# liron88/HM-16.2

Hardware: AMD Instinct MI355X
Metric: CTUs/sec (enc) at 4K main10; bit-exact CU partition vs HM (higher is better)
Workload: dtype int32+f64

## Files before the change

### hm-16.2_amd/csrc/hm355.hip

```cpp
#include <hip/hip_runtime.h>
#include <stdio.h>
#include <stdlib.h>
#include <string.h>
#include <memory>
#include <string>
#include <vector>
#include "hm355_core.h"
#include "hm355_dbk.h"
#include "hm355_sao.h"
#include "hm355_bits_kernel.h"
#include "hm355_ingest.h"
#include "hm355_picstat.h"
#include "hm355_host_common.h"
#include "../../include/hm355.h"

#define HM_SPIN_TIMEOUT_TICKS (40ull * 100000000ull)
typedef __attribute__((address_space(1))) unsigned int gu32;

__device__ __attribute__((noinline)) int hm355_wait_flag(const unsigned int *flag, unsigned int *abortWord, unsigned int epoch)
{
  int bad = 0;
  if (hm_lane() == 0) {
    const gu32 *f = (const gu32 *)flag; gu32 *ab = (gu32 *)abortWord;
    unsigned long long t0 = wall_clock64();
    unsigned int seen = __hip_atomic_load(ab + 1, __ATOMIC_RELAXED, __HIP_MEMORY_SCOPE_AGENT);
    while (__hip_atomic_load(f, __ATOMIC_RELAXED, __HIP_MEMORY_SCOPE_AGENT) != epoch) {
      __builtin_amdgcn_s_sleep(32);
      int stop = __hip_atomic_load(ab, __ATOMIC_RELAXED, __HIP_MEMORY_SCOPE_AGENT) != 0u;
      if (!stop && wall_clock64() - t0 > HM_SPIN_TIMEOUT_TICKS) {
        const unsigned int now = __hip_atomic_load(ab + 1, __ATOMIC_RELAXED, __HIP_MEMORY_SCOPE_AGENT);
        if (now != seen) { seen = now; t0 = wall_clock64(); } else stop = 1;
      }
      if (stop) {
        __hip_atomic_store(ab, 1u, __ATOMIC_RELAXED, __HIP_MEMORY_SCOPE_AGENT);
        bad = 1; break;
      }
    }
  }
  return __shfl(bad, 0, 64);
}

extern "C" __global__ void __launch_bounds__(64 * HM_CTU_WAVES, 3) hm355_ctu_kernel(const Params *P, const WorkItem *items, int total, unsigned int *sched, unsigned int epoch)
{
  __shared__ WorkItem curItems[HM_CTU_WAVES];
  const int wave = __builtin_amdgcn_readfirstlane((int)(threadIdx.x >> 6));
  if (wave == 0) load_tables();
  __syncthreads();
  WorkItem &curItem = curItems[wave];
  for (;;) {
    int idx = 0;
    if (hm_lane() == 0) idx = (int)atomicAdd(&sched[0], 1u);
    idx = __shfl(idx, 0, 64);
    if (idx >= total) break;
    if (hm_lane() == 0) curItem = items[idx];
    HM_SYNC();
    const int cx = curItem.ctuX, cy = curItem.ctuY, wCtu = P->wCtu;
    const unsigned int *done = P->frames[curItem.frame].done;
    const int a = cy * wCtu + cx;
    int dep0 = -1, dep1 = -1;
    if (P->wpp) {
      if (cx > 0) dep0 = a - 1;
      if (cy > 0) dep1 = (cy - 1) * wCtu + (cx + 1 < wCtu ? cx + 1 : cx);
    } else if (a > 0) dep0 = a - 1;
    const int dep2 = (P->wpp && cx == 0 && cy > 0 && P->frames[curItem.frame].imeta && (63 >= P->width || cy * 64 + 63 >= P->height)) ? a - 1 : -1;
    int bad = 0;
    if (dep0 >= 0) bad = hm355_wait_flag(done + dep0, sched + 1, epoch);
    if (!bad && dep1 >= 0) bad = hm355_wait_flag(done + dep1, sched + 1, epoch);
    if (!bad && dep2 >= 0) bad = hm355_wait_flag(done + dep2, sched + 1, epoch);
    if (bad) break;
    __builtin_amdgcn_fence(__ATOMIC_ACQUIRE, "agent");
    process_ctu(&g_shs[wave], P, &curItem, (int)blockIdx.x * HM_CTU_WAVES + wave);
    __builtin_amdgcn_fence(__ATOMIC_RELEASE, "agent");
    asm volatile("s_waitcnt vmcnt(0) lgkmcnt(0)" ::: "memory");
    if (hm_lane() == 0) { __hip_atomic_store((gu32 *)(done + a), epoch, __ATOMIC_RELAXED, __HIP_MEMORY_SCOPE_AGENT); __hip_atomic_fetch_add((gu32 *)(sched + 2), 1u, __ATOMIC_RELAXED, __HIP_MEMORY_SCOPE_AGENT); }
    HM_SYNC();
  }
}

extern "C" __global__ void __launch_bounds__(64 * HM_TEAM, 3) hm355_ctu_team_kernel(const Params *P, const WorkItem *items, int total, unsigned int *sched, unsigned int epoch)
{
  Team *T = HM_TEAM_PTR();
  const int wave = __builtin_amdgcn_readfirstlane((int)(threadIdx.x >> 6));
  if (threadIdx.x < HM_TEAM - 1) { T->box[threadIdx.x].reqSeq = 0; T->box[threadIdx.x].doneSeq = 0; }
  if (threadIdx.x == 0) { T->quit = 0; T->dead = 0; T->abortWord = sched + 1; T->waves = (int)(blockDim.x >> 6); }
  if (wave == 0) load_tables();
  __syncthreads();
  if (wave != 0) {
    team_helper(T, wave, wave <= HM_TEAM_HELPERS ? P->teamWin + ((size_t)blockIdx.x * HM_TEAM_HELPERS + (size_t)(wave - 1)) * P->teamWinStride : (Pel *)0);
    return;
  }
  for (;;) {
    int idx = 0;
    if (threadIdx.x == 0) idx = (int)atomicAdd(&sched[0], 1u);
    idx = __shfl(idx, 0, 64);
    if (idx >= total) break;
    if (threadIdx.x == 0) T->item = items[idx];
    HM_SYNC();
    const int cx = T->item.ctuX, cy = T->item.ctuY, wCtu = P->wCtu;
    const unsigned int *done = P->frames[T->item.frame].done;
    const int a = cy * wCtu + cx;
    int dep0 = -1, dep1 = -1;
    if (P->wpp) {
      if (cx > 0) dep0 = a - 1;
      if (cy > 0) dep1 = (cy - 1) * wCtu + (cx + 1 < wCtu ? cx + 1 : cx);
    } else if (a > 0) dep0 = a - 1;
    const int dep2 = (P->wpp && cx == 0 && cy > 0 && P->frames[T->item.frame].imeta && (63 >= P->width || cy * 64 + 63 >= P->height)) ? a - 1 : -1;
    int bad = 0;
    if (dep0 >= 0) bad = hm355_wait_flag(done + dep0, sched + 1, epoch);
    if (!bad && dep1 >= 0) bad = hm355_wait_flag(done + dep1, sched + 1, epoch);
    if (!bad && dep2 >= 0) bad = hm355_wait_flag(done + dep2, sched + 1, epoch);
    if (bad) break;
    __builtin_amdgcn_fence(__ATOMIC_ACQUIRE, "agent");
    process_ctu(&T->sh[0], P, &T->item, (int)blockIdx.x * T->waves, T);
    __builtin_amdgcn_fence(__ATOMIC_RELEASE, "agent");
    asm volatile("s_waitcnt vmcnt(0) lgkmcnt(0)" ::: "memory");
    if (threadIdx.x == 0) { __hip_atomic_store((gu32 *)(done + a), epoch, __ATOMIC_RELAXED, __HIP_MEMORY_SCOPE_AGENT); __hip_atomic_fetch_add((gu32 *)(sched + 2), 1u, __ATOMIC_RELAXED, __HIP_MEMORY_SCOPE_AGENT); }
    HM_SYNC();
    if (team_ld(&T->dead)) break;
  }
  HM_TEAM_RELEASE();
  team_st(&T->quit, 1u);
}

extern "C" __global__ void __launch_bounds__(64) hm355_dist_kernel(int kind, int n, int bitDepth, int count, const Pel *org, const Pel *cur, uint32_t *out)
{
  for (int b = (int)blockIdx.x; b < count; b += (int)gridDim.x) {
    const Pel *o = org + (size_t)b * n * n, *c = cur + (size_t)b * n * n;
    uint32_t v;
    if (kind == 0) v = dist_sad(o, n, c, n, n, 0, bitDepth);
    else if (kind == 3) v = dist_sad(o, n, c, n, n, 1, bitDepth);
    else if (kind == 1) v = dist_sse(o, n, c, n, n, bitDepth);
    else v = dist_hads(o, n, c, n, n, bitDepth);
    if (hm_lane() == 0) out[b] = v;
  }
}
extern "C" __global__ void __launch_bounds__(64) hm355_transform_kernel(int inverse, int n, int bitDepth, int useDst, int count, const int32_t *in, int32_t *out)
{
  Shared &sh = g_sh;
  load_tables();
  const int l2 = hm_log2(n);
  for (int b = (int)blockIdx.x; b < count; b += (int)gridDim.x) {
    const int32_t *src = in + (size_t)b * n * n; int32_t *dst = out + (size_t)b * n * n;
    HM_PAR_FOR(i, n * n) sh.bufA[(i >> l2) * HM_TSTRIDE + (i & (n - 1))] = src[i];
    HM_SYNC();
    if (inverse) inv_transform(&sh, n, useDst, bitDepth); else fwd_transform(&sh, n, useDst, bitDepth);
    HM_PAR_FOR(i, n * n) dst[i] = sh.bufA[(i >> l2) * HM_TSTRIDE + (i & (n - 1))];
    HM_SYNC();
  }
}

template <class T> struct DevBuf {
  T *p = nullptr; size_t n = 0;
  DevBuf() = default;
  DevBuf(DevBuf &&o) noexcept : p(o.p), n(o.n) { o.p = nullptr; o.n = 0; }
  DevBuf(const DevBuf &) = delete; DevBuf &operator=(const DevBuf &) = delete;
  ~DevBuf() { reset(); }
  operator T *() const { return p; }
  void reset() { if (p) (void)hipFree(p); p = nullptr; n = 0; }
  hipError_t alloc(size_t count)
  {
    reset();
    const hipError_t e = hipMalloc((void **)&p, count * sizeof(T));
    if (e == hipSuccess) n = count; else p = nullptr;
    return e;
  }
  hipError_t ensure(size_t count, bool zero = false)
  {
    if (p) return hipSuccess;
    const hipError_t e = alloc(count);
    return e == hipSuccess && zero ? hipMemset(p, 0, count * sizeof(T)) : e;
  }
  hipError_t grow(size_t count) { return count > n ? alloc(count) : hipSuccess; }
};
struct PinnedBuf {
  unsigned char *p = nullptr; size_t n = 0;
  PinnedBuf() = default;
  PinnedBuf(const PinnedBuf &) = delete; PinnedBuf &operator=(const PinnedBuf &) = delete;
  ~PinnedBuf() { reset(); }
  void reset() { if (p) (void)hipHostFree(p); p = nullptr; n = 0; }
  hipError_t grow(size_t bytes)
  {
    if (bytes <= n) return hipSuccess;
    reset();
    const hipError_t e = hipHostMalloc((void **)&p, bytes, hipHostMallocDefault);
    if (e == hipSuccess) n = bytes; else p = nullptr;
    return e;
  }
};
static size_t align256(size_t bytes) { return (bytes + 255) & ~(size_t)255; }

enum RefBuf { REF_Y, REF_CB, REF_CR, REF_PRED_MODE, REF_MV0, REF_REF_IDX0, REF_MV1, REF_REF_IDX1, REF_NBUF };
struct hm355_ref {
  RefPicDev dev = {};
  DevBuf<uint8_t> buf[REF_NBUF];
};
struct Slot {
  FrameBuf fb = {};
  DevBuf<InterMeta> imeta;
  DevBuf<Pel> saoSrc[3]; DevBuf<SaoStat> saoStat; DevBuf<SaoCand> saoCand; DevBuf<SaoBlk> saoCoded, saoRecon;
  DevBuf<uint8_t> rawIn, rawOut;
  DevBuf<uint8_t> bitsRaw, bitsPacked; DevBuf<uint32_t> bitsSizes; DevBuf<CabacW> bitsSync; DevBuf<uint32_t> bitsFlag; DevBuf<InterPic> bitsIp;
  DevBuf<DqpPic> dDqp; DevBuf<int8_t> dCtuQp; DevBuf<CtuDqp> dDqpOut; DevBuf<uint8_t> dRowFlag; int dqpOn = 0, dqpFlagIn = 0;
  std::vector<int8_t> ctuQp; std::vector<uint8_t> rowFlag; hm355_slice_desc lastSlice = {};
  std::vector<double> rcLambda; std::vector<CtuRc> rc; DevBuf<CtuRc> dRc; DevBuf<CtuRcOut> dRcOut;
  int sliceOpen = 0, ctusDone = 0, rcSearched = 0; int32_t firstCtu = 0; DevBuf<InterPic> dIp; DevBuf<MvD> dIntMv;
  int motionSet = 0; uint32_t motionSad = 0, motionSse = 0;
};
#define HM_QP_SLICE ((int8_t)-128)
#define HM_BITS_CAP_PER_CTU 16384u
#define HM_MAX_LANES 4
struct Lane {
  hipStream_t stream = NULL; hipEvent_t ev0 = NULL, ev1 = NULL;
  DevBuf<Params> dP;
  DevBuf<WorkSpace> dWs;
  DevBuf<WorkItem> dItems;
  DevBuf<unsigned int> dSched;
  std::vector<WorkItem> items; std::vector<int> stepStart; std::vector<FrameBuf> fbs;
  long long key[5] = {}; int keyValid = 0, fewWaves = -1;
  int busy = 0, grid = 0, inFixup = 0, prepared = 0;
  DevBuf<Pel> dTeamWin; size_t teamCap = 0;
  ~Lane() { if (ev0) (void)hipEventDestroy(ev0); if (ev1) (void)hipEventDestroy(ev1); if (stream) (void)hipStreamDestroy(stream); }
};
struct hm355_ctx {
  hm355_seq_cfg cfg = {};
  Params hp;
  DevBuf<Tables> dTab;
  DevBuf<FrameBuf> dFrames;
  DevBuf<uint8_t> arena;
  DevBuf<unsigned long long> prof;
  int teamLdsSet = 0;
  PinnedBuf hStage;
  unsigned int epoch = 0;
  std::vector<Slot> slots;
  Lane lane[HM_MAX_LANES];
  double lastKernelMs = 0; int lastLaunches = 0, laneShare = 1;
  std::string err;
  int numCtus = 0;
  DevBuf<DbkParams> dDbk;
  DevBuf<SaoParams> dSao;
  DevBuf<BitsParams> dBits;
  DevBuf<IngestParams> dIngest;
  DevBuf<int32_t> dIntraCost;
  DevBuf<PicStatParams> dPicStat; DevBuf<PicStatAcc> dPicAcc;
};

#define HM_CHECK(ctx, call) do { hipError_t e_ = (call); if (e_ != hipSuccess) { (ctx)->err = std::string(#call) + ": " + hipGetErrorString(e_); return HM355_ERR_DEVICE; } } while (0)

static int fail(hm355_ctx *c, int code, const char *msg) { if (c) c->err = msg; return code; }
static void next_epoch(hm355_ctx *c) { c->epoch++; if (c->epoch == 0) c->epoch = 1; }

#ifndef HM355_BUILD_ID
#define HM355_BUILD_ID "unknown"
#endif
extern "C" const char *hm355_build_id(void) { return HM355_BUILD_ID; }
extern "C" const char *hm355_last_error(const hm355_ctx *ctx) { return ctx ? ctx->err.c_str() : "no context"; }

static int maxItemsPerStep(int wCtu, int hCtu, int wpp, int frames)
{
  if (!wpp) return frames;
  int best = 0;
  for (int s = 0; s < wCtu + 2 * (hCtu - 1); s++) { int c = 0; for (int y = 0; y < hCtu; y++) { int x = s - 2 * y; if (x >= 0 && x < wCtu) c++; } if (c > best) best = c; }
  return best * frames;
}

static int lane_init(hm355_ctx *c, int l)
{
  Lane &L = c->lane[l];
  if (L.stream) return HM355_OK;
  HM_CHECK(c, l == 0 ? hipStreamCreate(&L.stream) : hipStreamCreateWithFlags(&L.stream, hipStreamNonBlocking));
  HM_CHECK(c, hipEventCreate(&L.ev0)); HM_CHECK(c, hipEventCreate(&L.ev1));
  size_t wsCount = (size_t)c->numCtus * (size_t)c->cfg.max_batch * HM_TEAM; if (wsCount > 3072) wsCount = 3072;
  HM_CHECK(c, L.dWs.alloc(wsCount));
  HM_CHECK(c, L.dSched.ensure(16, true));
  HM_CHECK(c, L.dP.alloc(1));
  return HM355_OK;
}

extern "C" int hm355_create(const hm355_seq_cfg *cfg, hm355_ctx **out)
{
  if (!cfg || !out) return HM355_ERR_ARG;
  *out = NULL;
  if (cfg->width <= 0 || cfg->height <= 0 || (cfg->width & 7) || (cfg->height & 7) || (cfg->bit_depth != 8 && cfg->bit_depth != 10) ||
      cfg->ctu_size != 64 || cfg->max_cu_depth != 4 || cfg->tu_log2_max != 5 || cfg->tu_log2_min != 2 || cfg->tu_max_depth_intra != 3 ||
      cfg->max_batch < 1 || (cfg->wavefront_synchro != 0 && cfg->wavefront_synchro != 1))
    return HM355_ERR_ARG;
  int ndev = 0;
  if (hipGetDeviceCount(&ndev) != hipSuccess || ndev <= 0) return HM355_ERR_NO_DEVICE;
  hm355_ctx *c = new hm355_ctx();
  c->cfg = *cfg;
  Params &P = c->hp; memset(&P, 0, sizeof(P));
  P.width = cfg->width; P.height = cfg->height; P.bitDepth = cfg->bit_depth; P.wpp = cfg->wavefront_synchro;
  P.wCtu = (cfg->width + 63) / 64; P.hCtu = (cfg->height + 63) / 64;
  P.stride[0] = P.wCtu * 64; P.stride[1] = P.stride[2] = P.wCtu * 32;
  c->numCtus = P.wCtu * P.hCtu;
  *out = c;
  { const int rc = lane_init(c, 0); if (rc != HM355_OK) return rc; }
  Tables *ht = new Tables; hm355_build_tables(ht);
  hipError_t e = c->dTab.alloc(1);
  if (e == hipSuccess) e = hipMemcpy(c->dTab, ht, sizeof(Tables), hipMemcpyHostToDevice);
  delete ht;
  HM_CHECK(c, e);
  HM_CHECK(c, c->dFrames.alloc(cfg->max_batch));
  c->slots.resize(cfg->max_batch);
  {
    size_t planeBytes[3], off = 0;
    for (int k = 0; k < 3; k++) planeBytes[k] = align256((size_t)P.stride[k] * P.hCtu * (k ? 32 : 64) * sizeof(Pel));
    const size_t metaBytes = align256(sizeof(CtuMeta) * c->numCtus), coefBytes = align256(sizeof(TCoeff) * (size_t)c->numCtus * HM_COEF_CTU);
    const size_t statBytes = align256(sizeof(CtuStat) * c->numCtus), endBytes = align256(sizeof(Cabac) * c->numCtus);
    const size_t doneBytes = align256(sizeof(uint32_t) * c->numCtus);
    const size_t slotBytes = 2 * (planeBytes[0] + planeBytes[1] + planeBytes[2]) + metaBytes + coefBytes + statBytes + endBytes + doneBytes;
    size_t freeB = 0, totalB = 0;
    if (hipMemGetInfo(&freeB, &totalB) == hipSuccess && slotBytes * (size_t)cfg->max_batch > freeB) {
      c->err = "hm355_create: max_batch pictures of this size do not fit the device memory"; return HM355_ERR_NOMEM; }
    HM_CHECK(c, c->arena.alloc(slotBytes * (size_t)cfg->max_batch));
    HM_CHECK(c, hipMemset(c->arena, 0, slotBytes * (size_t)cfg->max_batch));
    for (int s = 0; s < cfg->max_batch; s++) {
      FrameBuf &fb = c->slots[s].fb;
      uint8_t *p = c->arena + off;
      for (int k = 0; k < 3; k++) { fb.org[k] = (Pel *)p; p += planeBytes[k]; fb.rec[k] = (Pel *)p; p += planeBytes[k]; }
      fb.meta = (CtuMeta *)p; p += metaBytes; fb.coef = (TCoeff *)p; p += coefBytes; fb.stat = (CtuStat *)p; p += statBytes;
      fb.endState = (Cabac *)p; p += endBytes; fb.done = (uint32_t *)p; p += doneBytes;
      off += slotBytes;
    }
  }
  P.tab = c->dTab; P.ws = c->lane[0].dWs; P.frames = c->dFrames;
#ifdef HM355_PROFILE
  HM_CHECK(c, c->prof.alloc(2 * HM_PROF_N)); HM_CHECK(c, hipMemset(c->prof, 0, 2 * HM_PROF_N * sizeof(unsigned long long)));
  P.prof = c->prof;
#elif defined(HM355_TRACE)
  HM_CHECK(c, c->prof.alloc(1 + 3 * (size_t)HM_TRACE_CAP)); HM_CHECK(c, hipMemset(c->prof, 0, sizeof(unsigned long long)));
  P.prof = c->prof;
#endif
  HM_CHECK(c, hipMemcpy(c->lane[0].dP, &P, sizeof(Params), hipMemcpyHostToDevice));
  c->lane[0].fewWaves = P.fewWaves;
  return HM355_OK;
}

extern "C" void hm355_destroy(hm355_ctx *c)
{
  if (!c) return;
  for (int l = 0; l < HM_MAX_LANES; l++) if (c->lane[l].busy) (void)hipStreamSynchronize(c->lane[l].stream);
  delete c;
}

static hipError_t copy_planes(hm355_ctx *c, Pel *const dev[3], uint16_t *const host[3], hipMemcpyKind kind, bool async)
{
  const Params &P = c->hp;
  const bool up = kind == hipMemcpyHostToDevice;
  hipError_t e = hipSuccess;
  for (int k = 0; k < 3 && e == hipSuccess; k++) {
    const int w = P.width >> (k ? 1 : 0), h = P.height >> (k ? 1 : 0);
    const size_t devPitch = (size_t)P.stride[k] * sizeof(Pel), hostPitch = (size_t)w * 2;
    void *dst = up ? (void *)dev[k] : (void *)host[k]; const void *src = up ? (const void *)host[k] : (const void *)dev[k];
    const size_t dpitch = up ? devPitch : hostPitch, spitch = up ? hostPitch : devPitch;
    e = async ? hipMemcpy2DAsync(dst, dpitch, src, spitch, hostPitch, h, kind, c->lane[0].stream) : hipMemcpy2D(dst, dpitch, src, spitch, hostPitch, h, kind);
  }
  return e;
}

extern "C" int hm355_upload(hm355_ctx *c, int slot, const hm355_planes *org)
{
  if (!c || !org || slot < 0 || slot >= (int)c->slots.size()) return HM355_ERR_ARG;
  for (int k = 0; k < 3; k++) if (!org->plane[k]) return fail(c, HM355_ERR_ARG, "null plane");
  HM_CHECK(c, copy_planes(c, c->slots[slot].fb.org, org->plane, hipMemcpyHostToDevice, true));
  HM_CHECK(c, hipStreamSynchronize(c->lane[0].stream));
  c->slots[slot].ctusDone = 0;
  return HM355_OK;
}

static CtuRc slot_rc_record(const hm355_ctx *c, const Slot &sl, int qp, double lambda)
{
  CtuRc r = hm355_ctu_rc_record(c->hp.bitDepth, qp, lambda > 0 ? lambda : sl.lastSlice.lambda, sl.lastSlice.chroma_weight);
  if (!(lambda > 0) && sl.motionSet) { r.lambdaMotionSAD = sl.motionSad; r.lambdaMotionSSE = sl.motionSse; }
  return r;
}
static int dqp_prepare(hm355_ctx *c, int slot, const hm355_slice_desc *sd, hipStream_t stream, int resident)
{
  Slot &sl = c->slots[slot]; const Params &P = c->hp;
  sl.lastSlice = *sd;
  if (!sl.dqpOn) { sl.fb.dqp = NULL; return HM355_OK; }
  HM_CHECK(c, sl.dDqp.ensure(1)); HM_CHECK(c, sl.dCtuQp.ensure(c->numCtus));
  HM_CHECK(c, sl.dDqpOut.ensure(c->numCtus)); HM_CHECK(c, sl.dRowFlag.ensure(P.hCtu)); HM_CHECK(c, sl.dRcOut.ensure(c->numCtus));
  DqpPic *hp = new DqpPic; memset(hp, 0, sizeof(*hp));
  hp->flagIn = sl.dqpFlagIn; hp->sliceQp = sd->qp; hp->ctuQp = sl.dCtuQp; hp->out = sl.dDqpOut; hp->rowFlag = sl.dRowFlag;
  hp->rcOut = sl.dRcOut; hp->firstCtu = 0;
  hm355_fill_qp_tab(hp->tab, P.bitDepth, sd->lambda, sd->chroma_weight);
  std::vector<int8_t> q(c->numCtus, (int8_t)sd->qp);
  if (!sl.ctuQp.empty()) for (int a = 0; a < c->numCtus; a++) if (sl.ctuQp[a] != HM_QP_SLICE) q[a] = sl.ctuQp[a];
  int anyLambda = 0;
  for (size_t a = 0; a < sl.rcLambda.size(); a++) anyLambda |= sl.rcLambda[a] > 0;
  if (resident || anyLambda) {
    if (sl.dRc.ensure(c->numCtus) != hipSuccess) { delete hp; c->err = "hm355: out of device memory for the rate control records"; return HM355_ERR_NOMEM; }
    sl.rc.resize(c->numCtus);
    for (int a = 0; a < c->numCtus; a++)
      sl.rc[a] = slot_rc_record(c, sl, q[a], (size_t)a < sl.rcLambda.size() ? sl.rcLambda[a] : 0.0);
    hp->rc = sl.dRc;
  }
  hipError_t e1 = hipMemcpyAsync(sl.dDqp, hp, sizeof(DqpPic), hipMemcpyHostToDevice, stream);
  if (e1 == hipSuccess && hp->rc) e1 = hipMemcpyAsync(sl.dRc, sl.rc.data(), sizeof(CtuRc) * c->numCtus, hipMemcpyHostToDevice, stream);
  if (e1 == hipSuccess) e1 = hipMemcpyAsync(sl.dCtuQp, q.data(), c->numCtus, hipMemcpyHostToDevice, stream);
  if (e1 == hipSuccess) e1 = hipMemcpyAsync(sl.dRowFlag, sl.rowFlag.data(), P.hCtu, hipMemcpyHostToDevice, stream);
  if (e1 == hipSuccess) e1 = hipStreamSynchronize(stream);
  delete hp;
  HM_CHECK(c, e1);
  sl.fb.dqp = sl.dDqp;
  return HM355_OK;
}

static int run_begin(hm355_ctx *c, int l, int slot0, int n, const hm355_slice_desc *slices, int ctu0, int ctu1)
{
  const Params &P = c->hp;
  int rc = lane_init(c, l);
  if (rc != HM355_OK) return rc;
  Lane &L = c->lane[l];
  if (L.busy) return fail(c, HM355_ERR_ARG, "hm355_run_begin: the lane still has a launch in flight (hm355_run_wait first)");
  L.fbs.resize(n);
  for (int f = 0; f < n; f++) {
    if (slices) {
      if (slices[f].slice_type != 2) return fail(c, HM355_ERR_ARG, "only I slices are supported");
      if (slices[f].qp < 0 || slices[f].qp > 51 || !(slices[f].lambda > 0) || !(slices[f].chroma_weight > 0)) return fail(c, HM355_ERR_ARG, "bad slice parameters");
      hm355_fill_slice_params(&c->slots[slot0 + f].fb, P.bitDepth, slices[f].qp, slices[f].lambda, slices[f].chroma_weight);
      { const int rc2 = dqp_prepare(c, slot0 + f, slices + f, L.stream, c->slots[slot0 + f].sliceOpen); if (rc2 != HM355_OK) return rc2; }
    }
    L.fbs[f] = c->slots[slot0 + f].fb;
  }
  HM_CHECK(c, hipMemcpyAsync(c->dFrames + slot0, L.fbs.data(), sizeof(FrameBuf) * n, hipMemcpyHostToDevice, L.stream));
  int carry = 0;
  for (int f = 0; f < n; f++) carry |= c->slots[slot0 + f].fb.imeta != NULL && (P.height & 63) != 0;
  const long long key[5] = {slot0, n, carry, ctu0, ctu1};
  if (!L.keyValid || memcmp(key, L.key, sizeof(key)) != 0) {
    L.keyValid = 0;
    hm355_build_schedule(P.wCtu, P.hCtu, P.wpp, n, L.items, L.stepStart, carry, slot0, ctu0, ctu1);
    HM_CHECK(c, L.dItems.grow(L.items.size()));
    HM_CHECK(c, hipMemcpyAsync(L.dItems, L.items.data(), sizeof(WorkItem) * L.items.size(), hipMemcpyHostToDevice, L.stream));
    memcpy(L.key, key, sizeof(key)); L.keyValid = 1;
  }
  const long long parallel = (long long)n * (P.wpp ? 16 : 1);
  const int fewWaves = parallel < 1280 ? 1 : 0;
  const size_t wsCount = L.dWs.n;
  int anyInter = 0;
  for (int f = 0; f < n; f++) if (c->slots[slot0 + f].fb.imeta) anyInter = 1;
  int useTeam = (anyInter ? (P.wpp ? n <= 96 : n <= 1024) : parallel <= 512) && wsCount >= HM_TEAM;
  { const char *ev = getenv("HM355_TEAM"); if (ev && ev[0] == '0') useTeam = 0; if (ev && ev[0] == '1' && wsCount >= HM_TEAM) useTeam = 1; }
  const size_t winSamples = (size_t)65 * P.stride[0] + (size_t)33 * (P.stride[1] + P.stride[2]);
  int teams = 0;
  int waves = anyInter ? HM_TEAM : HM_TEAM_I;
  { const char *ev = getenv("HM355_TEAM_WAVES"); if (ev && atoi(ev) == HM_TEAM_I) waves = HM_TEAM_I; }
  if (useTeam) {
    const size_t total = L.items.size();
    const int rows = ctu1 / P.wCtu - ctu0 / P.wCtu + 1;
    size_t want = (size_t)maxItemsPerStep(P.wCtu, rows < P.hCtu ? rows : P.hCtu, P.wpp, n) + 2;
    if (want > total) want = total; if (want > 512) want = 512; if (want > wsCount / waves) want = wsCount / waves;
    if (want > L.teamCap) {
      HM_CHECK(c, hipStreamSynchronize(L.stream));
      L.teamCap = 0; L.fewWaves = -1;
      if (L.dTeamWin.alloc(want * HM_TEAM_HELPERS * winSamples) != hipSuccess) { (void)hipGetLastError(); useTeam = 0; }
      else L.teamCap = want;
    }
    teams = (int)(want < L.teamCap ? want : L.teamCap);
  }
  if (fewWaves != L.fewWaves) {
    Params lp = c->hp; lp.ws = L.dWs; lp.fewWaves = fewWaves; lp.teamWin = L.dTeamWin; lp.teamWinStride = winSamples;
    if (l == 0) { c->hp.fewWaves = fewWaves; c->hp.teamWin = L.dTeamWin; c->hp.teamWinStride = winSamples; }
    HM_CHECK(c, hipMemcpyAsync(L.dP, &lp, sizeof(Params), hipMemcpyHostToDevice, L.stream));
    HM_CHECK(c, hipStreamSynchronize(L.stream));
    L.fewWaves = fewWaves;
  }
  next_epoch(c);
  HM_CHECK(c, hipMemsetAsync(L.dSched, 0, 32, L.stream));
  if (ctu0 > 0)
    for (int f = 0; f < n; f++) HM_CHECK(c, hipMemsetD32Async((hipDeviceptr_t)c->slots[slot0 + f].fb.done, (int)c->epoch, ctu0, L.stream));
  L.prepared = slices == NULL;
  HM_CHECK(c, hipEventRecord(L.ev0, L.stream));
  const int total = (int)L.items.size();
  if (useTeam && teams > 0) {
    L.grid = teams;
    const size_t lds = HM_TEAM_LDS_BYTES(waves);
    if (!c->teamLdsSet) { HM_CHECK(c, hipFuncSetAttribute((const void *)hm355_ctu_team_kernel, hipFuncAttributeMaxDynamicSharedMemorySize, (int)HM_TEAM_LDS_BYTES(HM_TEAM))); c->teamLdsSet = 1; }
    hipLaunchKernelGGL(hm355_ctu_team_kernel, dim3(L.grid), dim3(64 * waves), lds, L.stream, (const Params *)L.dP, (const WorkItem *)L.dItems, total, L.dSched, c->epoch);
  } else {
    L.grid = total < (int)wsCount ? total : (int)wsCount;
    if (c->laneShare > 1) { const int cap = (int)(3072 * 5 / (4 * c->laneShare)); if (L.grid > cap) L.grid = cap; }
    int groups = (L.grid + HM_CTU_WAVES - 1) / HM_CTU_WAVES;
    if (groups > (int)(wsCount / HM_CTU_WAVES)) groups = (int)(wsCount / HM_CTU_WAVES);
    L.grid = groups * HM_CTU_WAVES;
    hipLaunchKernelGGL(hm355_ctu_kernel, dim3(groups), dim3(64 * HM_CTU_WAVES), 0, L.stream, (const Params *)L.dP, (const WorkItem *)L.dItems, total, L.dSched, c->epoch);
  }
  HM_CHECK(c, hipGetLastError());
  HM_CHECK(c, hipEventRecord(L.ev1, L.stream));
  L.busy = 1;
  return HM355_OK;
}
static int run_wait(hm355_ctx *c, int l, double *kernelMs);
static int dqp_verify_rows(hm355_ctx *c, int l, int slot0, int n, int ctu0, int ctu1, int prepared)
{
  const Params &P = c->hp;
  if (!P.wpp || P.wCtu < 1) return HM355_OK;
  for (int f = 0; f < n; f++) {
    Slot &sl = c->slots[slot0 + f];
    if (!sl.dqpOn || !sl.fb.dqp) continue;
    const int firstGuess = prepared ? (sl.firstCtu > ctu0 ? sl.firstCtu : ctu0) + 1 : 1;
    const int yLo = (firstGuess + P.wCtu - 1) / P.wCtu, yHi = ctu1 / P.wCtu;
    std::vector<CtuDqp> out(c->numCtus);
    for (int y = yLo < 1 ? 1 : yLo; y <= yHi; y++) {
      HM_CHECK(c, hipMemcpy(out.data(), sl.dDqpOut, sizeof(CtuDqp) * c->numCtus, hipMemcpyDeviceToHost));
      int bad = -1;
      for (int yy = y; yy <= yHi; yy++) if (sl.rowFlag[yy] != out[(size_t)yy * P.wCtu - 1].flagOut) { bad = yy; break; }
      if (bad < 0) break;
      sl.rowFlag[bad] = out[(size_t)bad * P.wCtu - 1].flagOut;
      const hm355_slice_desc sd = sl.lastSlice;
      int rc = HM355_OK;
      if (prepared) rc = hipMemcpyAsync(sl.dRowFlag.p + bad, &sl.rowFlag[bad], 1, hipMemcpyHostToDevice, c->lane[l].stream) == hipSuccess ? HM355_OK : fail(c, HM355_ERR_DEVICE, "row flag upload failed");
      if (rc == HM355_OK) rc = run_begin(c, l, slot0 + f, 1, prepared ? NULL : &sd, bad * P.wCtu, ctu1);
      if (rc == HM355_OK) rc = run_wait(c, l, NULL);
      if (rc != HM355_OK) return rc;
      y = bad;
    }
  }
  return HM355_OK;
}
static int run_wait(hm355_ctx *c, int l, double *kernelMs)
{
  Lane &L = c->lane[l];
  if (!L.busy) return fail(c, HM355_ERR_ARG, "hm355_run_wait: no launch in flight on this lane");
  L.busy = 0;
  HM_CHECK(c, hipStreamSynchronize(L.stream));
  float ms = 0; HM_CHECK(c, hipEventElapsedTime(&ms, L.ev0, L.ev1));
  unsigned int sched[2] = {0, 0};
  HM_CHECK(c, hipMemcpyAsync(sched, L.dSched, sizeof(sched), hipMemcpyDeviceToHost, L.stream));
  HM_CHECK(c, hipStreamSynchronize(L.stream));
#if defined(HM355_TEAMSTAT)
  { unsigned int ts[8] = {0}; (void)hipMemcpy(ts, L.dSched, sizeof(ts), hipMemcpyDeviceToHost);
    if (ts[3]) fprintf(stderr, "[team] CTUs %u: main wavefront %.1f ms/CTU = 8x8 CUs %.1f + waiting for helpers %.1f + rest; re-searched CUs %u\n",
                       ts[3], ts[4] * 1.28e-3 / ts[3], ts[6] * 1.28e-3 / ts[3], ts[5] * 1.28e-3 / ts[3], ts[7]); }
#endif
  if (sched[1] != 0) return fail(c, HM355_ERR_DEVICE, "scheduler aborted: a dependency wait timed out");
  c->lastKernelMs = ms; c->lastLaunches = 1;
  if (kernelMs) *kernelMs = ms;
  if (L.keyValid && !L.inFixup) {
    const int slot0 = (int)L.key[0], n = (int)L.key[1], ctu1 = (int)L.key[4];
    L.inFixup = 1;
    const int rc = dqp_verify_rows(c, l, slot0, n, (int)L.key[3], ctu1, L.prepared);
    L.inFixup = 0; L.keyValid = 0;
    c->lastKernelMs = ms;
    if (rc != HM355_OK) return rc;
    for (int f = 0; f < n; f++) {
      Slot &sl = c->slots[slot0 + f];
      sl.ctusDone = ctu1 + 1; sl.rcSearched = sl.fb.dqp != NULL;
    }
  }
  return HM355_OK;
}
static int run_rows_impl(hm355_ctx *c, int slot0, int n, const hm355_slice_desc *slices, int row0, int row1)
{
  const int rc = run_begin(c, 0, slot0, n, slices, row0 * c->hp.wCtu, (row1 + 1) * c->hp.wCtu - 1);
  return rc != HM355_OK ? rc : run_wait(c, 0, NULL);
}

extern "C" int hm355_run_begin(hm355_ctx *c, int lane, int first_slot, int n, const hm355_slice_desc *slices)
{
  if (!c || !slices || lane < 0 || lane >= HM_MAX_LANES || n < 1 || first_slot < 0 || first_slot + n > (int)c->slots.size()) return HM355_ERR_ARG;
  for (int f = 0; f < n; f++) if (c->slots[first_slot + f].fb.imeta) return fail(c, HM355_ERR_ARG, "hm355_run_begin: I slices only");
  for (int l = 0; l < HM_MAX_LANES; l++)
    if (l != lane && c->lane[l].busy && c->lane[l].keyValid && first_slot < (int)(c->lane[l].key[0] + c->lane[l].key[1]) && (int)c->lane[l].key[0] < first_slot + n)
      return fail(c, HM355_ERR_ARG, "hm355_run_begin: the slots overlap a launch in flight on another lane");
  return run_begin(c, lane, first_slot, n, slices, 0, c->numCtus - 1);
}
extern "C" int hm355_set_lane_share(hm355_ctx *c, int launches_in_flight)
{
  if (!c || launches_in_flight < 1 || launches_in_flight > HM_MAX_LANES) return HM355_ERR_ARG;
  c->laneShare = launches_in_flight;
  return HM355_OK;
}
extern "C" int hm355_run_wait(hm355_ctx *c, int lane, double *kernel_ms)
{
  if (!c || lane < 0 || lane >= HM_MAX_LANES) return HM355_ERR_ARG;
  return run_wait(c, lane, kernel_ms);
}

template <class F> static int timed_launches(hm355_ctx *c, int launches, F enqueue)
{
  Lane &L = c->lane[0];
  HM_CHECK(c, hipEventRecord(L.ev0, L.stream));
  HM_CHECK(c, enqueue(L.stream));
  HM_CHECK(c, hipEventRecord(L.ev1, L.stream));
  HM_CHECK(c, hipStreamSynchronize(L.stream));
  float ms = 0; HM_CHECK(c, hipEventElapsedTime(&ms, L.ev0, L.ev1));
  c->lastKernelMs = ms; c->lastLaunches = launches;
  return HM355_OK;
}
template <class T> static int stage_slots(hm355_ctx *c, const std::vector<FrameBuf> &fbs, DevBuf<T> &dst, const std::vector<T> &params)
{
  const hipStream_t s = c->lane[0].stream;
  HM_CHECK(c, dst.ensure(c->slots.size()));
  HM_CHECK(c, hipMemcpyAsync(c->dFrames, fbs.data(), sizeof(FrameBuf) * fbs.size(), hipMemcpyHostToDevice, s));
  HM_CHECK(c, hipMemcpyAsync(dst, params.data(), sizeof(T) * fbs.size(), hipMemcpyHostToDevice, s));
  HM_CHECK(c, hipStreamSynchronize(s));
  return HM355_OK;
}

extern "C" int hm355_set_dqp(hm355_ctx *c, int slot, const hm355_dqp_desc *d)
{
  if (!c || slot < 0 || slot >= (int)c->slots.size()) return HM355_ERR_ARG;
  Slot &sl = c->slots[slot];
  if (sl.sliceOpen) return fail(c, HM355_ERR_ARG, "hm355_set_dqp: a slice is open on the slot (hm355_slice_end first)");
  sl.rcLambda.clear();
  if (!d || !d->use_dqp) { sl.dqpOn = 0; sl.fb.dqp = NULL; sl.ctuQp.clear(); return HM355_OK; }
  const int lo = -6 * (c->hp.bitDepth - 8);
  sl.ctuQp.clear();
  if (d->ctu_qp) {
    for (int a = 0; a < c->numCtus; a++) if (d->ctu_qp[a] < lo || d->ctu_qp[a] > 51) return fail(c, HM355_ERR_ARG, "hm355_set_dqp: CTU QP out of range");
    sl.ctuQp.assign(d->ctu_qp, d->ctu_qp + c->numCtus);
  }
  sl.dqpOn = 1; sl.dqpFlagIn = d->dqp_flag_in != 0;
  sl.rowFlag.assign(c->hp.hCtu, 0);
  return HM355_OK;
}
extern "C" int hm355_get_dqp(hm355_ctx *c, int slot, int8_t *qp_out, int32_t *dqp_flag_out)
{
  if (!c || slot < 0 || slot >= (int)c->slots.size()) return HM355_ERR_ARG;
  Slot &sl = c->slots[slot];
  if (!sl.dqpOn || !sl.dDqpOut) return fail(c, HM355_ERR_ARG, "hm355_get_dqp: the slot was not searched with cu_qp_delta");
  std::vector<CtuDqp> out(c->numCtus);
  HM_CHECK(c, hipMemcpy(out.data(), sl.dDqpOut, sizeof(CtuDqp) * c->numCtus, hipMemcpyDeviceToHost));
  if (qp_out) for (int a = 0; a < c->numCtus; a++) for (int z = 0; z < 256; z++) qp_out[(size_t)a * 256 + z] = z < out[a].firstZ ? out[a].refQp : out[a].qp;
  if (dqp_flag_out) *dqp_flag_out = out[c->numCtus - 1].flagOut;
  return HM355_OK;
}
extern "C" int hm355_preanalyze(hm355_ctx *c, int slot, uint64_t *sums)
{
  if (!c || !sums || slot < 0 || slot >= (int)c->slots.size()) return HM355_ERR_ARG;
  DevBuf<unsigned long long> d;
  HM_CHECK(c, hipMemcpy(c->dFrames + slot, &c->slots[slot].fb, sizeof(FrameBuf), hipMemcpyHostToDevice));
  HM_CHECK(c, d.alloc((size_t)8 * c->numCtus));
  const Params *dP = c->lane[0].dP;
  const int rc = timed_launches(c, 1, [&](hipStream_t s) {
    hipLaunchKernelGGL(hm355_preanalyze_kernel, dim3(c->numCtus), dim3(64), 0, s, dP, slot, d.p);
    return hipGetLastError();
  });
  if (rc != HM355_OK) return rc;
  HM_CHECK(c, hipMemcpy(sums, d, sizeof(unsigned long long) * d.n, hipMemcpyDeviceToHost));
  return HM355_OK;
}

static int inter_desc_check(hm355_ctx *c, const hm355_inter_slice_desc *sd, const char *who)
{
  const int isB = sd->base.slice_type == 0;
  if (sd->base.slice_type != 1 && !isB) return fail(c, HM355_ERR_ARG, (std::string(who) + ": P (1) or B (0) slices").c_str());
  if (sd->num_ref_idx[0] < 1 || sd->num_ref_idx[0] > 16 || (isB ? (sd->num_ref_idx[1] < 1 || sd->num_ref_idx[1] > 16) : sd->num_ref_idx[1] != 0) ||
      sd->max_merge_cand < 1 || sd->max_merge_cand > 5 || (sd->cabac_init_type != 0 && sd->cabac_init_type != 1) ||
      sd->col_ref_idx < 0 || sd->col_ref_idx >= sd->num_ref_idx[(isB && !sd->col_from_l0) ? 1 : 0])
    return fail(c, HM355_ERR_ARG, "bad inter slice parameters");
  return HM355_OK;
}
static void inter_pic_params(const hm355_inter_slice_desc *sd, InterPic *ip)
{
  memset(ip, 0, sizeof(*ip));
  ip->sliceType = sd->base.slice_type; ip->poc = sd->poc; ip->numRefIdx[0] = sd->num_ref_idx[0]; ip->numRefIdx[1] = sd->num_ref_idx[1];
  ip->colFromL0 = sd->col_from_l0; ip->colRefIdx = sd->col_ref_idx; ip->tmvp = sd->tmvp; ip->mvdL1Zero = sd->mvd_l1_zero;
  ip->maxMergeCand = sd->max_merge_cand; ip->checkLDC = sd->check_ldc; ip->cabacInitType = sd->cabac_init_type;
  ip->lambdaMotionSAD = sd->lambda_motion_sad; ip->lambdaMotionSSE = sd->lambda_motion_sse;
}
static void inter_pic_list1(const hm355_inter_slice_desc *sd, InterPic *ip)
{
  for (int i1 = 0; i1 < sd->num_ref_idx[1]; i1++) {
    ip->list1ToList0[i1] = -1;
    for (int i0 = 0; i0 < sd->num_ref_idx[0]; i0++) if (ip->ref[0][i0].poc == ip->ref[1][i1].poc) { ip->list1ToList0[i1] = i0; break; }
  }
}

static_assert(sizeof(hm355_ctu_rc) == sizeof(CtuRcOut), "hm355_ctu_rc mirrors CtuRcOut");
#define HM_RC_LAMBDA_MIN 1e-4
#define HM_RC_LAMBDA_MAX 65535.0
static bool open_slice_armed(const hm355_ctx *c, const Slot &sl) { return sl.fb.dqp && sl.rc.size() == (size_t)c->numCtus && sl.dRc && sl.dRcOut; }
extern "C" int hm355_set_ctu_rc(hm355_ctx *c, int slot, int first_ctu, int n, const int8_t *qp, const double *lambda)
{
  if (!c || slot < 0 || slot >= (int)c->slots.size()) return HM355_ERR_ARG;
  Slot &sl = c->slots[slot];
  if (!sl.dqpOn) return fail(c, HM355_ERR_ARG, "hm355_set_ctu_rc: the slot is not armed with cu_qp_delta (hm355_set_dqp with use_dqp 1 first)");
  if (!qp || n < 1 || first_ctu < 0 || first_ctu + n > c->numCtus) return fail(c, HM355_ERR_ARG, "hm355_set_ctu_rc: bad CTU range (or no QPs)");
  if (sl.sliceOpen && !open_slice_armed(c, sl)) return fail(c, HM355_ERR_ARG, "hm355_set_ctu_rc: the open slice was not begun on an armed slot");
  if (sl.sliceOpen && first_ctu < sl.ctusDone) return fail(c, HM355_ERR_ARG, "hm355_set_ctu_rc: those CTUs of the open slice are searched already");
  const int lo = -6 * (c->hp.bitDepth - 8);
  for (int i = 0; i < n; i++) {
    if (qp[i] < lo || qp[i] > 51) return fail(c, HM355_ERR_ARG, "hm355_set_ctu_rc: CTU QP outside [-QpBDOffset, 51]");
    if (lambda && !(lambda[i] >= HM_RC_LAMBDA_MIN && lambda[i] <= HM_RC_LAMBDA_MAX)) return fail(c, HM355_ERR_ARG, "hm355_set_ctu_rc: a lambda must lie in [1e-4, 65535]");
  }
  if (sl.ctuQp.empty()) sl.ctuQp.assign(c->numCtus, HM_QP_SLICE);
  if (sl.rcLambda.empty()) sl.rcLambda.assign(c->numCtus, 0.0);
  for (int i = 0; i < n; i++) { sl.ctuQp[first_ctu + i] = qp[i]; sl.rcLambda[first_ctu + i] = lambda ? lambda[i] : 0.0; }
  if (!sl.sliceOpen) return HM355_OK;
  for (int i = 0; i < n; i++) sl.rc[first_ctu + i] = slot_rc_record(c, sl, qp[i], lambda ? lambda[i] : 0.0);
  const hipStream_t s = c->lane[0].stream;
  HM_CHECK(c, hipMemcpyAsync(sl.dRc.p + first_ctu, sl.rc.data() + first_ctu, sizeof(CtuRc) * n, hipMemcpyHostToDevice, s));
  HM_CHECK(c, hipMemcpyAsync(sl.dCtuQp.p + first_ctu, sl.ctuQp.data() + first_ctu, (size_t)n, hipMemcpyHostToDevice, s));
  return HM355_OK;
}
// ... 772 lines not shown
```

### hm-16.2_amd/csrc/hm355_host_common.h

```cpp
#pragma once
#include "hm355_types.h"
#include <math.h>
#include <string.h>
#include <vector>

static inline void hm355_gen_scan(int w, int h, int stride, int type, int offx, int offy, uint16_t *out, int count)
{
  int line = 0, col = 0;
  for (int i = 0; i < count; i++) {
    out[i] = (uint16_t)((line + offy) * stride + col + offx);
    if (type == 0) {
      if (col == w - 1 || line == 0) { line += col + 1; col = 0; if (line >= h) { col += line - (h - 1); line = h - 1; } }
      else { col++; line--; }
    } else if (type == 1) { if (col == w - 1) { line++; col = 0; } else col++; }
    else { if (line == h - 1) { col++; line = 0; } else line++; }
  }
}
static inline void hm355_build_tables(Tables *t)
{
  memset(t, 0, sizeof(*t));
  for (int z = 0; z < 256; z++) {
    int x = 0, y = 0;
    for (int b = 0; b < 4; b++) { x |= ((z >> (2 * b)) & 1) << b; y |= ((z >> (2 * b + 1)) & 1) << b; }
    t->z2r[z] = (uint8_t)(y * 16 + x); t->r2z[y * 16 + x] = (uint8_t)z;
  }
  for (int ty = 0; ty < 3; ty++)
    for (int l = 0; l < 4; l++) {
      const int n = 4 << l, g = n >> 2;
      hm355_gen_scan(g, g, g, ty, 0, 0, t->scanCG[ty][l], g * g);
      for (int gi = 0; gi < g * g; gi++) {
        const int gx = t->scanCG[ty][l][gi] % g, gy = t->scanCG[ty][l][gi] / g;
        hm355_gen_scan(4, 4, n, ty, gx * 4, gy * 4, t->scan[ty][l] + gi * 16, 16);
      }
    }
}

static const uint8_t HM355_CHROMA_SCALE_420[58] = { 0, 1, 2, 3, 4, 5, 6, 7, 8, 9,10,11,12,13,14,15,16,17,18,19,20,21,22,23,24,25,26,27,28,29,29,30,31,32,33,33,34,34,35,35,36,36,37,37,38,39,40,41,42,43,44,45,46,47,48,49,50,51 };

static inline void hm355_fill_slice_params(FrameBuf *f, int bitDepth, int qp, double lambda, double chromaWeight)
{
  static const int quantScales[6] = {26214, 23302, 20560, 18396, 16384, 14564};
  static const int invQuantScales[6] = {40, 45, 51, 57, 64, 72};
  f->qp = qp; f->lambda = lambda; f->sqrtLambda = sqrt(lambda); f->chromaWeight = chromaWeight; f->lambdaC = lambda / chromaWeight;
  const int bdOff = 6 * (bitDepth - 8);
  const int q = qp + bdOff; f->qpPer[0] = q / 6; f->qpRem[0] = q % 6;
  int qc = qp < -bdOff ? -bdOff : (qp > 57 ? 57 : qp);
  qc = (qc < 0) ? qc + bdOff : HM355_CHROMA_SCALE_420[qc] + bdOff;
  f->qpPer[1] = qc / 6; f->qpRem[1] = qc % 6;
  for (int ch = 0; ch < 2; ch++) {
    for (int l = 0; l < 4; l++) {
      const int transformShift = 15 - bitDepth - (l + 2);
      double errScale = (double)(1 << 15);
      errScale = errScale * pow(2.0, -2.0 * transformShift);
      errScale = errScale / quantScales[f->qpRem[ch]] / quantScales[f->qpRem[ch]] / (double)(1 << (2 * (bitDepth - 8)));
      f->errScale[ch][l] = errScale;
    }
    const double lam = ch ? f->lambdaC : f->lambda;
    const double invQ = (double)invQuantScales[f->qpRem[ch]];
    f->rdFactor[ch] = (int64_t)(invQ * invQ * (double)(1 << (2 * f->qpPer[ch])) / lam / 16 / (double)(1 << (2 * (bitDepth - 8))) + 0.5);
  }
}

static inline void hm355_fill_qp_tab(QpTab tab[64], int bitDepth, double lambda, double chromaWeight)
{
  for (int q = -12; q <= 51; q++) {
    FrameBuf t; memset(&t, 0, sizeof(t));
    hm355_fill_slice_params(&t, bitDepth, q, lambda, chromaWeight);
    QpTab &e = tab[q + 12];
    for (int k = 0; k < 2; k++) { e.qpPer[k] = t.qpPer[k]; e.qpRem[k] = t.qpRem[k]; e.rdFactor[k] = t.rdFactor[k]; for (int l = 0; l < 4; l++) e.errScale[k][l] = t.errScale[k][l]; }
  }
}

static inline CtuRc hm355_ctu_rc_record(int bitDepth, int qp, double lambda, double chromaWeight)
{
  FrameBuf t; memset(&t, 0, sizeof(t));
  hm355_fill_slice_params(&t, bitDepth, qp, lambda, chromaWeight);
  CtuRc r; memset(&r, 0, sizeof(r));
  r.lambda = t.lambda; r.sqrtLambda = t.sqrtLambda; r.lambdaC = t.lambdaC; r.rdFactor[0] = t.rdFactor[0]; r.rdFactor[1] = t.rdFactor[1];
  r.lambdaMotionSAD = (uint32_t)floor(65536.0 * t.sqrtLambda); r.lambdaMotionSSE = (uint32_t)floor(65536.0 * lambda);
  return r;
}

static inline void hm355_intra_lambda(int qp, double *lambda, double *chromaWeight)
{
  *lambda = 0.57 * pow(2.0, ((double)qp - 12) / 3.0);
  const int q = qp < 0 ? 0 : (qp > 57 ? 57 : qp);
  const int qpc = HM355_CHROMA_SCALE_420[q];
  *chromaWeight = pow(2.0, (qp - qpc) / 3.0);
}

static inline int hm355_schedule_step(int wCtu, int hCtu, int wpp, int carryLastRow, int x, int y)
{
  if (!wpp) return y * wCtu + x;
  if (carryLastRow && hCtu > 1 && wCtu > 1 && y == hCtu - 1) return (wCtu - 1) + 2 * (hCtu - 2) + 1 + x;
  return x + 2 * y;
}
static inline void hm355_build_schedule(int wCtu, int hCtu, int wpp, int nFrames, std::vector<WorkItem> &items, std::vector<int> &stepStart, int carryLastRow = 0,
                                        int firstFrame = 0, int firstCtu = 0, int lastCtu = -1)
{
  items.clear(); stepStart.clear();
  if (lastCtu < 0) lastCtu = wCtu * hCtu - 1;
  const int steps = hm355_schedule_step(wCtu, hCtu, wpp, carryLastRow, wCtu - 1, hCtu - 1) + 1;
  std::vector<std::vector<WorkItem> > bucket(steps);
  for (int a = firstCtu; a <= lastCtu; a++) { const int x = a % wCtu, y = a / wCtu; WorkItem w = {0, x, y, 0}; bucket[hm355_schedule_step(wCtu, hCtu, wpp, carryLastRow, x, y)].push_back(w); }
  for (int s = 0; s < steps; s++) {
    stepStart.push_back((int)items.size());
    for (int f = 0; f < nFrames; f++) for (size_t i = 0; i < bucket[s].size(); i++) { WorkItem w = bucket[s][i]; w.frame = firstFrame + f; items.push_back(w); }
  }
  stepStart.push_back((int)items.size());
}
```

Baseline: 25220.

## Split WPP intra encode into team/wave/team phases for ramp-up and ramp-down

For all-intra WPP encodes, the work schedule is split into up to three launches. The narrow wavefront head and tail steps run on the team kernel, where multiple waves cooperate per CTU, and the wide middle runs on the one-wave-per-CTU kernel. This targets the idle hardware during WPP ramp-up and ramp-down, where few CTUs are ready at once and single-wave-per-CTU leaves most of the GPU unused. The scheduler also checks the abort word before claiming work. The cost is extra kernel launches and scheduler-counter resets between phases, plus a second Params buffer and team window allocation.

```diff
diff --git a/hm-16.2_amd/csrc/hm355.hip b/hm-16.2_amd/csrc/hm355.hip
--- a/hm-16.2_amd/csrc/hm355.hip
+++ b/hm-16.2_amd/csrc/hm355.hip
@@ -49,7 +49,7 @@
   WorkItem &curItem = curItems[wave];
   for (;;) {
     int idx = 0;
-    if (hm_lane() == 0) idx = (int)atomicAdd(&sched[0], 1u);
+    if (hm_lane() == 0) idx = __hip_atomic_load((gu32 *)(sched + 1), __ATOMIC_RELAXED, __HIP_MEMORY_SCOPE_AGENT) ? total : (int)atomicAdd(&sched[0], 1u);
     idx = __shfl(idx, 0, 64);
     if (idx >= total) break;
     if (hm_lane() == 0) curItem = items[idx];
@@ -91,7 +91,7 @@
   }
   for (;;) {
     int idx = 0;
-    if (threadIdx.x == 0) idx = (int)atomicAdd(&sched[0], 1u);
+    if (threadIdx.x == 0) idx = __hip_atomic_load((gu32 *)(sched + 1), __ATOMIC_RELAXED, __HIP_MEMORY_SCOPE_AGENT) ? total : (int)atomicAdd(&sched[0], 1u);
     idx = __shfl(idx, 0, 64);
     if (idx >= total) break;
     if (threadIdx.x == 0) T->item = items[idx];
@@ -209,15 +209,18 @@
 #define HM_QP_SLICE ((int8_t)-128)
 #define HM_BITS_CAP_PER_CTU 16384u
 #define HM_MAX_LANES 4
+#define HM355_RAMP_TEAM_CAP 512u
 struct Lane {
   hipStream_t stream = NULL; hipEvent_t ev0 = NULL, ev1 = NULL;
   DevBuf<Params> dP;
+  DevBuf<Params> dPTeam;
   DevBuf<WorkSpace> dWs;
   DevBuf<WorkItem> dItems;
   DevBuf<unsigned int> dSched;
   std::vector<WorkItem> items; std::vector<int> stepStart; std::vector<FrameBuf> fbs;
   long long key[5] = {}; int keyValid = 0, fewWaves = -1;
   int busy = 0, grid = 0, inFixup = 0, prepared = 0;
+  int launches = 1;
   DevBuf<Pel> dTeamWin; size_t teamCap = 0;
   ~Lane() { if (ev0) (void)hipEventDestroy(ev0); if (ev1) (void)hipEventDestroy(ev1); if (stream) (void)hipStreamDestroy(stream); }
 };
@@ -459,10 +462,36 @@
     }
     teams = (int)(want < L.teamCap ? want : L.teamCap);
   }
+  Hm355Phase phase[3]; int phases = 0, phaseTeams = 0, forced = -1;
+  { const char *ev = getenv("HM355_RAMP_TEAMS"); if (ev && ev[0]) forced = atoi(ev) > 0 ? atoi(ev) : 0; }
+  int rampOk = (!useTeam || forced > 0) && !anyInter && P.wpp && c->laneShare == 1 && wsCount / HM_TEAM_I > 0;
+  for (int f = 0; f < n && rampOk; f++) if (L.fbs[f].dqp) rampOk = 0;
+  { const char *ev = getenv("HM355_TEAM"); if (ev && ev[0] == '0') rampOk = 0; }
+  if (rampOk) {
+    size_t want = L.items.size();
+    if (want > HM355_RAMP_TEAM_CAP) want = HM355_RAMP_TEAM_CAP; if (want > wsCount / HM_TEAM_I) want = wsCount / HM_TEAM_I;
+    const int threshold = forced >= 0 ? forced : hm355_phase_default_threshold((int)want);
+    phases = hm355_plan_phases(L.stepStart, (int)want, threshold, phase, forced >= 0 ? 0.0 : HM355_PHASE_MIN_SAVED_STEPS);
+    if (useTeam && phases == 1) phases = 0;
+    if (phases == 1 && phase[0].mode == HM355_PHASE_WAVE) phases = 0;
+    if (phases && want > L.teamCap) {
+      HM_CHECK(c, hipStreamSynchronize(L.stream));
+      L.teamCap = 0; L.fewWaves = -1;
+      if (L.dTeamWin.alloc(want * HM_TEAM_HELPERS * winSamples) != hipSuccess) { (void)hipGetLastError(); phases = 0; useTeam = 0; teams = 0; }
+      else L.teamCap = want;
+    }
+    if (phases && !L.dPTeam) {
+      if (L.dPTeam.alloc(1) != hipSuccess) { (void)hipGetLastError(); phases = 0; }
+      L.fewWaves = -1;
+    }
+    phaseTeams = (int)want;
+  }
   if (fewWaves != L.fewWaves) {
     Params lp = c->hp; lp.ws = L.dWs; lp.fewWaves = fewWaves; lp.teamWin = L.dTeamWin; lp.teamWinStride = winSamples;
     if (l == 0) { c->hp.fewWaves = fewWaves; c->hp.teamWin = L.dTeamWin; c->hp.teamWinStride = winSamples; }
     HM_CHECK(c, hipMemcpyAsync(L.dP, &lp, sizeof(Params), hipMemcpyHostToDevice, L.stream));
+    lp.fewWaves = 1;
+    if (L.dPTeam) HM_CHECK(c, hipMemcpyAsync(L.dPTeam, &lp, sizeof(Params), hipMemcpyHostToDevice, L.stream));
     HM_CHECK(c, hipStreamSynchronize(L.stream));
     L.fewWaves = fewWaves;
   }
@@ -473,10 +502,29 @@
   L.prepared = slices == NULL;
   HM_CHECK(c, hipEventRecord(L.ev0, L.stream));
   const int total = (int)L.items.size();
-  if (useTeam && teams > 0) {
+  L.launches = 1;
+  if ((useTeam && teams > 0) || phases) {
+    if (!c->teamLdsSet) { HM_CHECK(c, hipFuncSetAttribute((const void *)hm355_ctu_team_kernel, hipFuncAttributeMaxDynamicSharedMemorySize, (int)HM_TEAM_LDS_BYTES(HM_TEAM))); c->teamLdsSet = 1; }
+  }
+  if (phases) {
+    L.launches = phases;
+    for (int k = 0; k < phases; k++) {
+      const WorkItem *first = L.dItems + phase[k].first; const int count = phase[k].count;
+      if (k > 0) HM_CHECK(c, hipMemsetAsync(L.dSched, 0, sizeof(unsigned int), L.stream));
+      if (phase[k].mode == HM355_PHASE_TEAM) {
+        L.grid = count < phaseTeams ? count : phaseTeams;
+        hipLaunchKernelGGL(hm355_ctu_team_kernel, dim3(L.grid), dim3(64 * HM_TEAM_I), HM_TEAM_LDS_BYTES(HM_TEAM_I), L.stream, (const Params *)L.dPTeam, first, count, L.dSched, c->epoch);
+      } else {
+        int groups = ((count < (int)wsCount ? count : (int)wsCount) + HM_CTU_WAVES - 1) / HM_CTU_WAVES;
+        if (groups > (int)(wsCount / HM_CTU_WAVES)) groups = (int)(wsCount / HM_CTU_WAVES);
+        L.grid = groups * HM_CTU_WAVES;
+        hipLaunchKernelGGL(hm355_ctu_kernel, dim3(groups), dim3(64 * HM_CTU_WAVES), 0, L.stream, (const Params *)L.dP, first, count, L.dSched, c->epoch);
+      }
+      HM_CHECK(c, hipGetLastError());
+    }
+  } else if (useTeam && teams > 0) {
     L.grid = teams;
     const size_t lds = HM_TEAM_LDS_BYTES(waves);
-    if (!c->teamLdsSet) { HM_CHECK(c, hipFuncSetAttribute((const void *)hm355_ctu_team_kernel, hipFuncAttributeMaxDynamicSharedMemorySize, (int)HM_TEAM_LDS_BYTES(HM_TEAM))); c->teamLdsSet = 1; }
     hipLaunchKernelGGL(hm355_ctu_team_kernel, dim3(L.grid), dim3(64 * waves), lds, L.stream, (const Params *)L.dP, (const WorkItem *)L.dItems, total, L.dSched, c->epoch);
   } else {
     L.grid = total < (int)wsCount ? total : (int)wsCount;
@@ -535,14 +583,15 @@
                        ts[3], ts[4] * 1.28e-3 / ts[3], ts[6] * 1.28e-3 / ts[3], ts[5] * 1.28e-3 / ts[3], ts[7]); }
 #endif
   if (sched[1] != 0) return fail(c, HM355_ERR_DEVICE, "scheduler aborted: a dependency wait timed out");
-  c->lastKernelMs = ms; c->lastLaunches = 1;
+  const int launches = L.launches;
+  c->lastKernelMs = ms; c->lastLaunches = launches;
   if (kernelMs) *kernelMs = ms;
   if (L.keyValid && !L.inFixup) {
     const int slot0 = (int)L.key[0], n = (int)L.key[1], ctu1 = (int)L.key[4];
     L.inFixup = 1;
     const int rc = dqp_verify_rows(c, l, slot0, n, (int)L.key[3], ctu1, L.prepared);
     L.inFixup = 0; L.keyValid = 0;
-    c->lastKernelMs = ms;
+    c->lastKernelMs = ms; c->lastLaunches = launches;
     if (rc != HM355_OK) return rc;
     for (int f = 0; f < n; f++) {
       Slot &sl = c->slots[slot0 + f];
diff --git a/hm-16.2_amd/csrc/hm355_host_common.h b/hm-16.2_amd/csrc/hm355_host_common.h
--- a/hm-16.2_amd/csrc/hm355_host_common.h
+++ b/hm-16.2_amd/csrc/hm355_host_common.h
@@ -109,3 +109,37 @@
   }
   stepStart.push_back((int)items.size());
 }
+
+enum { HM355_PHASE_WAVE = 0, HM355_PHASE_TEAM = 1 };
+struct Hm355Phase { int first, count, mode; };
+#define HM355_TEAM_STEP_RATIO 0.4
+#define HM355_PHASE_MIN_SAVED_STEPS 2.0
+static inline int hm355_phase_default_threshold(int teams) { return (int)(teams / HM355_TEAM_STEP_RATIO); }
+static inline double hm355_phase_saved_steps(const std::vector<int> &stepStart, int s0, int s1, int teams)
+{
+  double saved = 0;
+  for (int s = s0; s < s1; s++) {
+    const int c = stepStart[s + 1] - stepStart[s];
+    if (c > 0) saved += 1.0 - HM355_TEAM_STEP_RATIO * (c > teams ? (double)c / teams : 1.0);
+  }
+  return saved;
+}
+static inline int hm355_plan_phases(const std::vector<int> &stepStart, int teams, int threshold, Hm355Phase out[3], double minSavedSteps = HM355_PHASE_MIN_SAVED_STEPS)
+{
+  const int steps = (int)stepStart.size() - 1, total = steps >= 0 ? stepStart[steps] : 0;
+  int n = 0;
+  if (total <= 0) return 0;
+  int head = 0, tail = steps;
+  if (threshold > 0 && teams > 0) {
+    while (head < steps && stepStart[head + 1] - stepStart[head] <= threshold) head++;
+    while (tail > head && stepStart[tail] - stepStart[tail - 1] <= threshold) tail--;
+    if (head < steps) {
+      if (hm355_phase_saved_steps(stepStart, 0, head, teams) < minSavedSteps) head = 0;
+      if (hm355_phase_saved_steps(stepStart, tail, steps, teams) < minSavedSteps) tail = steps;
+    }
+  }
+  const int cut[4] = {0, stepStart[head], stepStart[tail], total};
+  for (int k = 0; k < 3; k++)
+    if (cut[k + 1] > cut[k]) { out[n].first = cut[k]; out[n].count = cut[k + 1] - cut[k]; out[n].mode = k == 1 ? HM355_PHASE_WAVE : HM355_PHASE_TEAM; n++; }
+  return n;
+}
```

New measurement: 26300, median of 6. +4.3%, better.
